# facebookresearch/vggsfm

Measured on NVIDIA H100. Metric: BA iterations/sec, higher is better.
Workload: dtype f64

## Files before the change

vggsfm_b200/csrc/ba_schur.cu:

```cuda
#include <stddef.h>
#include <algorithm>
#include <vector>
#include "ba_obs.h"
#include "common.cuh"
#include "dev_probes.h"
#include "syrk_work.h"

namespace vgg {

__device__ __forceinline__ void ar_add(double* local, double* mc, double v) {
  if (mc) asm volatile("multimem.red.relaxed.sys.global.add.f64 [%0], %1;" ::"l"(mc), "d"(v) : "memory");
  else atomicAdd(local, v);
}
__device__ __forceinline__ void ar_put(double* local, double* mc, double v) {
  if (mc) asm volatile("multimem.red.relaxed.sys.global.add.f64 [%0], %1;" ::"l"(mc), "d"(v) : "memory");
  else *local = v;
}

__global__ void jacobi_scale_points_kernel(int N, const double* __restrict__ H_pp, double* __restrict__ sc_p, int enable) {
  const int n = blockIdx.x * blockDim.x + threadIdx.x;
  if (n >= N) return;
  const double* h = H_pp + (size_t)n * 6;
  sc_p[n * 3 + 0] = enable ? 1.0 / (1.0 + sqrt(h[0])) : 1.0;
  sc_p[n * 3 + 1] = enable ? 1.0 / (1.0 + sqrt(h[3])) : 1.0;
// ... 29 lines not shown
  const double d2 = fmin(fmax(v22, min_diag), max_diag);
  dpp[n * 3] = d0; dpp[n * 3 + 1] = d1; dpp[n * 3 + 2] = d2;
  v00 += d0 / radius; v11 += d1 / radius; v22 += d2 / radius;
  bool bad = !(v00 > 0.0);
  const double l00 = sqrt(v00);
  const double l10 = v01 / l00, l20 = v02 / l00;
  const double t11 = v11 - l10 * l10;
  bad = bad || !(t11 > 0.0);
  const double l11 = sqrt(t11);
  const double l21 = (v12 - l20 * l10) / l11;
  const double t22 = v22 - l20 * l20 - l21 * l21;
  bad = bad || !(t22 > 0.0);
  const double l22 = sqrt(t22);
  if (bad) {
    atomicAdd(&scal[6], 1.0);
#pragma unroll
    for (int i = 0; i < 9; ++i) Mo[i] = 0.0;
    q[n * 3] = q[n * 3 + 1] = q[n * 3 + 2] = 0.0;
    return;
  }
  const double i00 = 1.0 / l00, i11 = 1.0 / l11, i22 = 1.0 / l22;
  const double i10 = -l10 * i00 * i11;
  const double i21 = -l21 * i11 * i22;
  const double i20 = -(l20 * i00 + l21 * i10) * i22;
  const double m00 = s0 * i00, m01 = s0 * i10, m02 = s0 * i20;
  const double m11 = s1 * i11, m12 = s1 * i21;
  const double m22 = s2 * i22;
  Mo[0] = m00; Mo[1] = m01; Mo[2] = m02;
  Mo[3] = 0.0; Mo[4] = m11; Mo[5] = m12;
  Mo[6] = 0.0; Mo[7] = 0.0; Mo[8] = m22;
  const double g0 = g_p[n * 3], g1 = g_p[n * 3 + 1], g2 = g_p[n * 3 + 2];
  q[n * 3 + 0] = m00 * g0;
  q[n * 3 + 1] = m01 * g0 + m11 * g1;
  q[n * 3 + 2] = m02 * g0 + m12 * g1 + m22 * g2;
}

__global__ void assemble_hc_kernel(int S, int dc, int ns, int KR, int Dpad, const double* __restrict__ camrec,
                                   const double* __restrict__ shared_in, double* __restrict__ Sraw,
                                   double* __restrict__ rhs, double* __restrict__ hdiag, double* __restrict__ gvec,
                                   ptrdiff_t mc_off) {
  const int s = blockIdx.x;
  const int tid = threadIdx.x;
#define VGG_PUT(ptr, val) ar_put((ptr), mc_off ? (ptr) + mc_off : nullptr, (val))
  if (s < S) {
    const double* rec = camrec + (size_t)s * KR;
    const int base = s * dc;
    if (tid < dc) {
      VGG_PUT(&gvec[base + tid], rec[tid]);
      VGG_PUT(&rhs[base + tid], -rec[tid]);
    }
    if (tid < dc * dc) {
      const int i = tid / dc, j = tid % dc;
      const int a = i < j ? i : j, b = i < j ? j : i;
      const int idx = dc + a * dc - a * (a - 1) / 2 + (b - a);
      const double val = rec[idx];
      VGG_PUT(&Sraw[(size_t)(base + i) * Dpad + base + j], val);
      if (i == j) VGG_PUT(&hdiag[base + i], val);
    }
    if (tid < 6 * ns) {
      const int i = tid / ns, j = tid % ns;
      const double val = rec[dc + dc * (dc + 1) / 2 + tid];
      VGG_PUT(&Sraw[(size_t)(S * dc + j) * Dpad + base + i], val);
      VGG_PUT(&Sraw[(size_t)(base + i) * Dpad + S * dc + j], val);
    }
  } else if (ns > 0) {
    const int base = S * dc;
    if (tid < ns) {
      VGG_PUT(&gvec[base + tid], shared_in[tid]);
      VGG_PUT(&rhs[base + tid], -shared_in[tid]);
    }
    if (tid < ns * ns) {
      const int i = tid / ns, j = tid % ns;
      const int a = i < j ? i : j, b = i < j ? j : i;
      const double val = shared_in[2 + (a == 0 ? b : 2)];
      VGG_PUT(&Sraw[(size_t)(base + i) * Dpad + base + j], val);
      if (i == j) VGG_PUT(&hdiag[base + i], val);
    }
  }
#undef VGG_PUT
}

constexpr int ZB_NT = 8;
constexpr int ZB_W = 4;
template <int MODEL, int MODE>
__global__ void __launch_bounds__(ZB_W * 32) z_build_kernel(
    int S, int N, int Dpad, const float* __restrict__ uv, const uint8_t* __restrict__ mask,
    const double* __restrict__ poses, const double* __restrict__ intr, const double* __restrict__ points,
    const uint8_t* __restrict__ point_const, const double* __restrict__ M, const double* __restrict__ q,
    double* __restrict__ Zt, double* __restrict__ rhs, ptrdiff_t mc_off, const int* __restrict__ fg_tracks) {
  using C = BlkCfg<MODEL, MODE>;
  constexpr int DC = C::DC, NS = C::NS;
  constexpr int ZR = 32 * DC;
  __shared__ __align__(16) double s_cam[ZB_W][16 * 32];
  __shared__ __align__(16) double s_z[ZB_W][3 * ZR];
  __shared__ double s_pt[ZB_NT][16];
  __shared__ double s_ws[ZB_W][ZB_NT][3 * (NS > 0 ? NS : 1)];
  const int lane = threadIdx.x & 31, warp = threadIdx.x >> 5;
  const int n0 = blockIdx.x * ZB_NT, nt = min(ZB_NT, N - n0);
  const int ngroups = (S + 31) / 32;
  for (int e = threadIdx.x; e < ZB_NT * 16; e += blockDim.x) {
    const int t = e >> 4, k = e & 15, n = n0 + t;
    double v = 0.0;
    if (t < nt) {
      if (k < 3) v = points[(size_t)n * 3 + k];
      else if (k == 3) v = (point_const && point_const[n]) ? 1.0 : 0.0;
      else if (k < 13) v = M[(size_t)n * 9 + (k - 4)];
      else v = q[(size_t)n * 3 + (k - 13)];
    }
    s_pt[t][k] = v;
  }
  if (NS > 0)
    for (int e = threadIdx.x; e < ZB_W * ZB_NT * 3 * NS; e += blockDim.x) (&s_ws[0][0][0])[e] = 0.0;
  __syncthreads();
  double* pw = s_cam[warp];
  double* zs = s_z[warp];
  const float2* uv2 = reinterpret_cast<const float2*>(uv);
  for (int g = warp; g < ngroups; g += ZB_W) {
    if (fg_tracks && (n0 + nt <= fg_tracks[2 * g] || n0 >= fg_tracks[2 * g + 1])) continue;
    const int s = g * 32 + lane;
    const bool frame_ok = s < S;
    const int cnt = min(32, S - g * 32) * DC;
    __syncwarp();
#pragma unroll
    for (int i = 0; i < 12; ++i) pw[i * 32 + lane] = frame_ok ? poses[(size_t)s * 12 + i] : 0.0;
#pragma unroll
    for (int i = 0; i < 4; ++i) pw[(12 + i) * 32 + lane] = frame_ok ? intr[(size_t)s * 4 + i] : 0.0;
    __syncwarp();
    double zq[DC];
#pragma unroll
    for (int i = 0; i < DC; ++i) zq[i] = 0.0;
    for (int t = 0; t < nt; ++t) {
      const size_t o = (size_t)s * N + n0 + t;
      const bool valid = frame_ok && mask[o] != 0;
      if (!__any_sync(0xffffffffu, valid)) continue;
      const float2 ob = frame_ok ? uv2[o] : make_float2(0.f, 0.f);
      const double* pt = s_pt[t];
      const double* m = pt + 4;
      double jc0[8], jc1[8], jx0[3], jx1[3], rx, ry;
      obs_math<MODEL>(pw + lane, 32, pt[0], pt[1], pt[2], pt[3] != 0.0, ob.x, ob.y, valid, jc0, jc1, jx0, jx1, rx, ry);
#pragma unroll
      for (int i = 0; i < DC; ++i) {
        const double w0 = w_entry(jc0, jc1, jx0, jx1, i, 0), w1 = w_entry(jc0, jc1, jx0, jx1, i, 1),
                     w2 = w_entry(jc0, jc1, jx0, jx1, i, 2);
        const double z0 = w0 * m[0];
        const double z1 = w0 * m[1] + w1 * m[4];
        const double z2 = w0 * m[2] + w1 * m[5] + w2 * m[8];
        zs[lane * DC + i] = z0;
        zs[ZR + lane * DC + i] = z1;
        zs[2 * ZR + lane * DC + i] = z2;
        zq[i] += z0 * m[9] + z1 * m[10] + z2 * m[11];
      }
      if (NS > 0) {
        double a[8];
#pragma unroll
        for (int k = 0; k < 8; ++k) a[k] = k < 3 * NS ? w_entry(jc0, jc1, jx0, jx1, 6 + k / 3, k % 3) : 0.0;
        const double r = warp_reduce_scatter<8>(a, lane);
        if (lane < 3 * NS) s_ws[warp][t][lane] += r;
      }
      __syncwarp();
      double* dst = Zt + (size_t)(3 * (n0 + t)) * Dpad + (size_t)g * ZR;
#pragma unroll
      for (int c = 0; c < 3; ++c, dst += Dpad) {
        const double* src = zs + c * ZR;
        for (int e = 2 * lane; e + 1 < cnt; e += 64)
          *reinterpret_cast<double2*>(dst + e) = *reinterpret_cast<const double2*>(src + e);
        if ((cnt & 1) && lane == 0) dst[cnt - 1] = src[cnt - 1];
      }
      __syncwarp();
    }
    if (frame_ok) {
#pragma unroll
      for (int i = 0; i < DC; ++i) {
        double* r = &rhs[(size_t)s * DC + i];
        if (zq[i] != 0.0) ar_add(r, mc_off ? r + mc_off : nullptr, zq[i]);
      }
    }
  }
  if (NS > 0) {
    __syncthreads();
    if ((int)threadIdx.x < nt * NS) {
      const int t = threadIdx.x / NS, j = threadIdx.x % NS;
      double w[3];
#pragma unroll
      for (int c = 0; c < 3; ++c) {
        w[c] = 0.0;
#pragma unroll
        for (int v = 0; v < ZB_W; ++v) w[c] += s_ws[v][t][j * 3 + c];
      }
      const double* m = s_pt[t] + 4;
      const double z0 = w[0] * m[0];
      const double z1 = w[0] * m[1] + w[1] * m[4];
      const double z2 = w[0] * m[2] + w[1] * m[5] + w[2] * m[8];
      double* zo = Zt + (size_t)(3 * (n0 + t)) * Dpad + (size_t)S * DC + j;
      zo[0] = z0;
      zo[Dpad] = z1;
      zo[2 * (size_t)Dpad] = z2;
      const double zq = z0 * m[9] + z1 * m[10] + z2 * m[11];
      double* r = &rhs[(size_t)S * DC + j];
      if (zq != 0.0) ar_add(r, mc_off ? r + mc_off : nullptr, zq);
    }
  }
}

constexpr int SF_BM = 128, SF_BK = 16, SF_LDS = 132, SF_STAGES = 4, SF_MMA_WARPS = 8;
constexpr int SF_THREADS = 128 + SF_MMA_WARPS * 32;
constexpr int SF_STAGE_DOUBLES = 2 * SF_BK * SF_LDS;
constexpr size_t SF_SMEM_BYTES = sizeof(double) * SF_STAGES * SF_STAGE_DOUBLES + sizeof(uint64_t) * 2 * SF_STAGES;

struct SyrkWork {
  int bi, bj, kb0, kb1;
};

__global__ void __launch_bounds__(SF_THREADS, 1)
    syrk_f64_kernel(const SyrkWork* __restrict__ work, int nwork, int Kpad, int Dpad, const double* __restrict__ Zt,
                    double* __restrict__ Cmat, ptrdiff_t mc_off, const __grid_constant__ FabricDev fd) {
  extern __shared__ __align__(16) double sf_smem[];
  uint64_t* full = reinterpret_cast<uint64_t*>(sf_smem + SF_STAGES * SF_STAGE_DOUBLES);
  uint64_t* empty = full + SF_STAGES;
  const int warp = threadIdx.x >> 5, lane = threadIdx.x & 31;
  if (threadIdx.x == 0) {
    for (int s = 0; s < SF_STAGES; ++s) {
      mbar_init(&full[s], 1);
      mbar_init(&empty[s], SF_MMA_WARPS);
    }
    mbar_fence_init();
  }
  __syncthreads();

  int stage = 0, phase = 0;
  if (warp < 4) {
    asm volatile("setmaxnreg.dec.sync.aligned.u32 40;");
    if (warp > 0) return;
    const int row = lane & (SF_BK - 1), opnd = lane / SF_BK;
    for (int w = blockIdx.x; w < nwork; w += gridDim.x) {
      const SyrkWork wk = work[w];
      const bool diag = wk.bi == wk.bj;
      const int k1 = min(Kpad, wk.kb1 * 64);
      for (int k = wk.kb0 * 64; k < k1; k += SF_BK) {
        mbar_wait(&empty[stage], phase ^ 1);
        if (lane == 0) mbar_expect_tx(&full[stage], (diag ? 1u : 2u) * SF_BK * SF_BM * (uint32_t)sizeof(double));
        __syncwarp();
        if (opnd == 0 || !diag)
          tma_load_1d(sf_smem + stage * SF_STAGE_DOUBLES + (opnd * SF_BK + row) * SF_LDS,
                      Zt + (size_t)(k + row) * Dpad + (opnd ? wk.bj : wk.bi) * SF_BM, SF_BM * sizeof(double), &full[stage]);
        if (++stage == SF_STAGES) {
          stage = 0;
          phase ^= 1;
        }
      }
    }
    return;
  }

  asm volatile("setmaxnreg.inc.sync.aligned.u32 232;");
  const int wm = (warp - 4) >> 2, wn = warp & 3;
  const int g = lane >> 2, t = lane & 3;
  for (int w = blockIdx.x; w < nwork; w += gridDim.x) {
// ... 220 lines not shown
      Q[i * 4 + j] = rot ? E[i * 3] * P[j] + E[i * 3 + 1] * P[4 + j] + E[i * 3 + 2] * P[8 + j] : P[i * 4 + j];
  Q[3] = d[3] != 0.0 ? P[3] + d[3] : P[3];
  Q[7] = d[4] != 0.0 ? P[7] + d[4] : P[7];
  Q[11] = d[5] != 0.0 ? P[11] + d[5] : P[11];
  const int ni = (model == VGG_SIMPLE_PINHOLE) ? 1 : 2;
  double f = intr[s * 4], k = intr[s * 4 + 3];
  const double* di = dc > 6 ? d + 6 : d_c + (size_t)S * dc;
  if (dc > 6 || ns > 0) {
    if (di[0] != 0.0) f += di[0];
    if (ni > 1 && di[1] != 0.0) k += di[1];
  }
  intr_c[s * 4] = f;
  intr_c[s * 4 + 1] = intr[s * 4 + 1];
  intr_c[s * 4 + 2] = intr[s * 4 + 2];
  intr_c[s * 4 + 3] = k;
}

__global__ void extract_gvec_kernel(int S, int dc, int ns, int KR, const double* __restrict__ camrec,
                                    const double* __restrict__ shared_in, double* __restrict__ gvec) {
  const int i = blockIdx.x * blockDim.x + threadIdx.x;
  const int D = S * dc + ns;
  if (i >= D) return;
  gvec[i] = (i < S * dc) ? camrec[(size_t)(i / dc) * KR + (i % dc)] : shared_in[i - S * dc];
}

__global__ void gradmax_kernel(int D, int N, const double* __restrict__ gvec, const uint8_t* __restrict__ pconst,
                               const double* __restrict__ g_p, const uint8_t* __restrict__ point_const,
                               double* __restrict__ scal) {
  const int i = blockIdx.x * blockDim.x + threadIdx.x;
  unsigned long long mc = 0, mp = 0;
  if (i < D && !pconst[i]) mc = (unsigned long long)__double_as_longlong(fabs(gvec[i]));
  if (i < N * 3 && !(point_const && point_const[i / 3])) mp = (unsigned long long)__double_as_longlong(fabs(g_p[i]));
#pragma unroll
  for (int off = 16; off >= 1; off >>= 1) {
    mc = max(mc, __shfl_xor_sync(0xffffffffu, mc, off));
    mp = max(mp, __shfl_xor_sync(0xffffffffu, mp, off));
  }
  if ((threadIdx.x & 31) == 0) {
    atomicMax(reinterpret_cast<unsigned long long*>(&scal[4]), mc);
    atomicMax(reinterpret_cast<unsigned long long*>(&scal[5]), mp);
  }
}

int launch_jacobi_scale_points(int N, const double* H_pp, double* sc_p, int enable, cudaStream_t st) {
  jacobi_scale_points_kernel<<<(N + 255) / 256, 256, 0, st>>>(N, H_pp, sc_p, enable);
  VGG_LAUNCH_CHECK();
  return VGG_OK;
}
int launch_jacobi_scale_cams(int D, const double* hdiag, double* sc_c, int enable, cudaStream_t st) {
  jacobi_scale_cams_kernel<<<(D + 255) / 256, 256, 0, st>>>(D, hdiag, sc_c, enable);
  VGG_LAUNCH_CHECK();
  return VGG_OK;
}
int launch_point_prep(int N, const double* H_pp, const double* g_p, const double* sc_p, const uint8_t* point_const,
                      double radius, double min_diag, double max_diag, double* M, double* q, double* dpp,
                      double* scal, cudaStream_t st) {
  point_prep_kernel<<<(N + 127) / 128, 128, 0, st>>>(N, H_pp, g_p, sc_p, point_const, radius, min_diag, max_diag, M, q,
                                                     dpp, scal);
  VGG_LAUNCH_CHECK();
  return VGG_OK;
}
int launch_assemble_hc(int S, int dc, int ns, int KR, int Dpad, const double* camrec, const double* shared_in,
                       double* Sraw, double* rhs, double* hdiag, double* gvec, ptrdiff_t mc_off, cudaStream_t st) {
  assemble_hc_kernel<<<S + (ns > 0 ? 1 : 0), 64, 0, st>>>(S, dc, ns, KR, Dpad, camrec, shared_in, Sraw, rhs, hdiag, gvec,
                                                          mc_off);
  VGG_LAUNCH_CHECK();
  return VGG_OK;
}
#define VGG_PICK_BA_KERNEL(kern, tmpl, p)                 \
  decltype(&tmpl<0, 0>) kern = nullptr;                   \
  switch ((p)->camera_model * 3 + (p)->intr_mode) {       \
    case 0: kern = tmpl<0, 0>; break;                     \
    case 1: kern = tmpl<0, 1>; break;                     \
    case 2: kern = tmpl<0, 2>; break;                     \
    case 3: kern = tmpl<1, 0>; break;                     \
    case 4: kern = tmpl<1, 1>; break;                     \
    case 5: kern = tmpl<1, 2>; break;                     \
  }                                                       \
  VGG_REQUIRE(kern, "bad camera_model/intr_mode")

int launch_z_build(const vgg_ba_problem* p, int Dpad, const double* M, const double* q, double* Zt, double* rhs,
                   ptrdiff_t mc_off, const int* fg_tracks, cudaStream_t st) {
  VGG_PICK_BA_KERNEL(kern, z_build_kernel, p);
  const int nw = std::min(ZB_W, (p->S + 31) / 32);
  kern<<<(p->N + ZB_NT - 1) / ZB_NT, nw * 32, 0, st>>>(p->S, p->N, Dpad, p->uv, p->mask, p->poses, p->intr, p->points,
                                                        p->point_const, M, q, Zt, rhs, mc_off, fg_tracks);
  VGG_LAUNCH_CHECK();
  return VGG_OK;
}

struct SyrkF64State {
  int dev = -1, Kpad = -1, Dpad = -1, sms = 0, nwork = 0;
  std::vector<int> ranges;
  SyrkWork* work_dev = nullptr;
  size_t work_cap = 0;
};
thread_local SyrkF64State g_sf;

static std::vector<SyrkWork> syrk_f64_work(int Kpad, int Dpad, const std::vector<int>& ranges, int nworkers) {
  const int nb = Dpad / SF_BM, KB = (Kpad + 63) / 64;
  std::vector<SyrkWork> work;
  build_work_list<SyrkWork>({1}, syrk_tile_jobs(nb, ranges), KB, nworkers, KB, 1,
                            [](const SyrkTileJob& j, int, int k0, int k1) { return SyrkWork{j.bi, j.bj, k0, k1}; }, &work);
  return work;
}

int launch_syrk(int Kpad, int Dpad, const double* Zt, double* Cmat, ptrdiff_t mc_off, const std::vector<int>& kb_ranges,
                const FabricDev& fd, cudaStream_t st) {
  VGG_REQUIRE(Dpad % SF_BM == 0 && Kpad % SF_BK == 0, "syrk: Dpad must be a multiple of 128 and Kpad of 16");
  const int nb = Dpad / SF_BM;
  SyrkF64State& hs = g_sf;
  const std::vector<int> ranges = (int)kb_ranges.size() == 2 * nb ? kb_ranges : std::vector<int>();
  int dev = 0;
  VGG_CUDA_CHECK(cudaGetDevice(&dev));
  if (hs.dev != dev || hs.Kpad != Kpad || hs.Dpad != Dpad || hs.ranges != ranges) {
    VGG_CUDA_CHECK(cudaDeviceGetAttribute(&hs.sms, cudaDevAttrMultiProcessorCount, dev));
    VGG_CUDA_CHECK(cudaFuncSetAttribute(syrk_f64_kernel, cudaFuncAttributeMaxDynamicSharedMemorySize, (int)SF_SMEM_BYTES));
    const std::vector<SyrkWork> work = syrk_f64_work(Kpad, Dpad, ranges, hs.sms);
    VGG_CUDA_CHECK(cudaDeviceSynchronize());
    if (hs.dev != dev || work.size() > hs.work_cap) {
      if (hs.work_dev) cudaFree(hs.work_dev);
      hs.work_dev = nullptr;
      hs.work_cap = std::max<size_t>(work.size(), 1);
      VGG_CUDA_CHECK(cudaMalloc(reinterpret_cast<void**>(&hs.work_dev), sizeof(SyrkWork) * hs.work_cap));
    }
    if (!work.empty())
      VGG_CUDA_CHECK(cudaMemcpy(hs.work_dev, work.data(), sizeof(SyrkWork) * work.size(), cudaMemcpyHostToDevice));
    hs.nwork = (int)work.size();
    hs.dev = dev;
    hs.Kpad = Kpad;
    hs.Dpad = Dpad;
    hs.ranges = ranges;
  }
  if (hs.nwork == 0) return VGG_OK;
  syrk_f64_kernel<<<std::min(hs.sms, hs.nwork), SF_THREADS, SF_SMEM_BYTES, st>>>(hs.work_dev, hs.nwork, Kpad, Dpad, Zt, Cmat,
                                                                               mc_off, fd);
  VGG_LAUNCH_CHECK();
  return VGG_OK;
}
int launch_scale_damp(int D, int Dpad, double* A, const double* rhs, const double* hdiag, const double* sc,
                      const uint8_t* pconst, double radius, double min_diag, double max_diag, double* bvec,
                      cudaStream_t st) {
  dim3 grid((D + 255) / 256, D);
  scale_damp_kernel<<<grid, 256, 0, st>>>(D, Dpad, A, rhs, hdiag, sc, pconst, radius, min_diag, max_diag, bvec);
  VGG_LAUNCH_CHECK();
  return VGG_OK;
}
int launch_cam_step(int D, const double* dcs, size_t dcs_stride, const double* sc, const double* hdiag, const double* gvec,
                    const uint8_t* pconst, double radius, double min_diag, double max_diag, double* d_c, double* scal,
                    cudaStream_t st) {
  cam_step_kernel<<<(D + 255) / 256, 256, 0, st>>>(D, dcs, dcs_stride, sc, hdiag, gvec, pconst, radius, min_diag, max_diag, d_c, scal);
  VGG_LAUNCH_CHECK();
  return VGG_OK;
}
int launch_backsub(const vgg_ba_problem* p, const double* d_c, double* wacc, const int* fg_tracks, cudaStream_t st) {
  VGG_PICK_BA_KERNEL(kern, backsub_kernel, p);
  const int nw = std::min(BS_W, p->S);
  kern<<<(p->N + 31) / 32, nw * 32, 0, st>>>(p->S, p->N, p->uv, p->mask, p->poses, p->intr, p->points, p->point_const,
                                             d_c, wacc, fg_tracks);
  VGG_LAUNCH_CHECK();
  return VGG_OK;
}
int launch_point_step(int N, const double* M, const double* g_p, const double* wacc, const double* sc_p,
                      const double* dpp, const uint8_t* point_const, const double* X, double radius, double* Xc,
                      double* scal, cudaStream_t st) {
  point_step_kernel<<<(N + 127) / 128, 128, 0, st>>>(N, M, g_p, wacc, sc_p, dpp, point_const, X, radius, Xc, scal);
  VGG_LAUNCH_CHECK();
  return VGG_OK;
// ... 61 lines not shown
```

vggsfm_b200/csrc/trsv.cu:

```cuda
#include "common.cuh"
#include "dev_probes.h"

namespace vgg {

namespace {

constexpr int TS_NB = 64;
constexpr int TS_THREADS = 256;
constexpr unsigned long long TS_SENTINEL = 0xffffffffffffffffull;

__global__ void __launch_bounds__(TS_THREADS, 1)
    trsv_upper_kernel(int n, int lda, const double* __restrict__ A, const double* __restrict__ y, size_t y_stride,
                      double* __restrict__ x, long long* __restrict__ stamps) {
  extern __shared__ __align__(16) double ts_smem[];
  double(*Ud)[TS_NB + 1] = reinterpret_cast<double(*)[TS_NB + 1]>(ts_smem);
  double(*Vi)[TS_NB + 1] = reinterpret_cast<double(*)[TS_NB + 1]>(ts_smem + TS_NB * (TS_NB + 1));
  double* xs = ts_smem + 2 * TS_NB * (TS_NB + 1);
  double* accs = xs + TS_NB;
  const int nb = gridDim.x;
  const int b = nb - 1 - (int)blockIdx.x;
  const int r0 = b * TS_NB;
  const int rows = min(TS_NB, n - r0);
  const int tid = threadIdx.x;
  const int r = tid >> 2, seg = tid & 3;
  auto stamp = [&](int k) {
    if (stamps && tid == 0) {
      long long t;
      asm volatile("mov.u64 %0, %%globaltimer;" : "=l"(t));
      stamps[6 * b + k] = t;
    }
  };
  stamp(0);
  double y_mine = 0.0;
  if (tid < TS_NB && tid < rows) y_mine = __ldcg(&y[(size_t)(r0 + tid) * y_stride]);

  for (int e = tid; e < TS_NB * TS_NB; e += TS_THREADS) {
    const int i = e / TS_NB, j = e % TS_NB;
    double v = (i == j) ? 1.0 : 0.0;
    if (i < rows && j < rows && j >= i) v = A[(size_t)(r0 + i) * lda + r0 + j];
    Ud[i][j] = v;
  }
  __syncthreads();
  stamp(1);
  if (tid < TS_NB) xs[tid] = 1.0 / Ud[tid][tid];
  __syncthreads();
  {
    const int c = tid >> 2, part = tid & 3;
    for (int i = TS_NB - 1; i >= 0; --i) {
      double s = 0.0;
      if (i < c) {
        for (int k = i + 1 + part; k <= c; k += 4) s = fma(-Ud[i][k], Vi[k][c], s);
      }
      s += __shfl_xor_sync(0xffffffffu, s, 1);
      s += __shfl_xor_sync(0xffffffffu, s, 2);
      if (part == 0) Vi[i][c] = i > c ? 0.0 : (i == c ? xs[i] : s * xs[i]);
      __syncwarp();
    }
  }
  __syncthreads();
  stamp(2);
  if (tid < TS_NB) accs[tid] = y_mine;
  __syncthreads();
  stamp(5);

  double t0[16], t1[16], t2[16];
  auto load_tile = [&](double (&tile)[16], int j) {
    const int c0 = j * TS_NB + seg * 16;
    const double* src = A + (size_t)(r0 + (r < rows ? r : 0)) * lda + c0;
#pragma unroll
    for (int k = 0; k < 16; ++k) tile[k] = (j > b && r < rows && c0 + k < n) ? src[k] : 0.0;
  };
  double acc = 0.0;
  auto hop = [&](const double (&tile)[16], int j) {
    if (tid < TS_NB) {
      double v = 0.0;
      if (j * TS_NB + tid < n) {
        const volatile unsigned long long* src = reinterpret_cast<const volatile unsigned long long*>(&x[j * TS_NB + tid]);
        unsigned long long bits;
        do {
          bits = *src;
        } while (bits == TS_SENTINEL);
        v = __longlong_as_double((long long)bits);
      }
      xs[tid] = v;
    }
    __syncthreads();
    double s0 = 0.0, s1 = 0.0, s2 = 0.0, s3 = 0.0;
#pragma unroll
    for (int k = 0; k < 16; k += 4) {
      s0 = fma(tile[k], xs[seg * 16 + k], s0);
      s1 = fma(tile[k + 1], xs[seg * 16 + k + 1], s1);
      s2 = fma(tile[k + 2], xs[seg * 16 + k + 2], s2);
      s3 = fma(tile[k + 3], xs[seg * 16 + k + 3], s3);
    }
    acc += (s0 + s1) + (s2 + s3);
    __syncthreads();
  };
  int j = nb - 1;
  if (b < nb - 1) {
  load_tile(t0, j);
  load_tile(t1, j - 1);
  load_tile(t2, j - 2);
  while (j > b) {
    hop(t0, j);
    load_tile(t0, j - 3);
    if (--j <= b) break;
    hop(t1, j);
    load_tile(t1, j - 3);
    if (--j <= b) break;
    hop(t2, j);
    load_tile(t2, j - 3);
    --j;
  }
  }
  stamp(3);
  acc += __shfl_xor_sync(0xffffffffu, acc, 1);
  acc += __shfl_xor_sync(0xffffffffu, acc, 2);
  if (seg == 0) accs[r] -= acc;
  __syncthreads();
  {
    double q0 = 0.0, q1 = 0.0, q2 = 0.0, q3 = 0.0;
#pragma unroll
    for (int k = 0; k < 16; k += 4) {
      const int c = seg * 16 + k;
      q0 = fma(c >= r ? Vi[r][c] : 0.0, accs[c], q0);
      q1 = fma(c + 1 >= r ? Vi[r][c + 1] : 0.0, accs[c + 1], q1);
      q2 = fma(c + 2 >= r ? Vi[r][c + 2] : 0.0, accs[c + 2], q2);
      q3 = fma(c + 3 >= r ? Vi[r][c + 3] : 0.0, accs[c + 3], q3);
    }
    double s = (q0 + q1) + (q2 + q3);
    s += __shfl_xor_sync(0xffffffffu, s, 1);
    s += __shfl_xor_sync(0xffffffffu, s, 2);
    if (seg == 0 && r < rows) {
      unsigned long long bits = (unsigned long long)__double_as_longlong(s);
      if (s != s) bits = 0x7ff8000000000000ull;
      *reinterpret_cast<volatile unsigned long long*>(&x[r0 + r]) = bits;
    }
  }
  if (stamps) {
    __syncthreads();
    stamp(4);
  }
}

}

int launch_trsv_upper(int n, int lda, const double* A, const double* y, size_t y_stride, double* x, long long* stamps,
                      cudaStream_t st) {
  const int nb = (n + TS_NB - 1) / TS_NB;
  VGG_REQUIRE(nb <= 120, "trsv_upper: n too large for one co-resident wave");
  const size_t smem = sizeof(double) * (2 * TS_NB * (TS_NB + 1) + 2 * TS_NB);
  static bool attr = false;
  if (!attr) {
    VGG_CUDA_CHECK(cudaFuncSetAttribute(trsv_upper_kernel, cudaFuncAttributeMaxDynamicSharedMemorySize, (int)smem));
    attr = true;
  }
  VGG_CUDA_CHECK(cudaMemsetAsync(x, 0xFF, sizeof(double) * (size_t)n, st));
  trsv_upper_kernel<<<nb, TS_THREADS, smem, st>>>(n, lda, A, y, y_stride, x, stamps);
  VGG_LAUNCH_CHECK();
  return VGG_OK;
}

}

extern "C" int vgg_dev_trsv_probe(int n, int lda, const double* A_dev, const double* y_dev, size_t y_stride, double* x_dev,
                                  long long* stamps_host) {
  using namespace vgg;
  VGG_REQUIRE(n > 0 && lda >= n && A_dev && y_dev && x_dev && y_stride > 0, "bad argument");
  const int nb = (n + TS_NB - 1) / TS_NB;
  static long long* d = nullptr;
  static int d_cap = 0;
  if (stamps_host && d_cap < 6 * nb) {
    if (d) cudaFree(d);
    VGG_CUDA_CHECK(cudaMalloc(&d, sizeof(long long) * 6 * nb));
    d_cap = 6 * nb;
  }
  if (stamps_host) VGG_CUDA_CHECK(cudaMemset(d, 0, sizeof(long long) * 6 * nb));
  const int rc = launch_trsv_upper(n, lda, A_dev, y_dev, y_stride, x_dev, stamps_host ? d : nullptr, 0);
  if (rc) return rc;
  VGG_CUDA_CHECK(cudaDeviceSynchronize());
  if (stamps_host) VGG_CUDA_CHECK(cudaMemcpy(stamps_host, d, sizeof(long long) * 6 * nb, cudaMemcpyDeviceToHost));
  return VGG_OK;
}
```

Before: 373.6.

## Rewrite TRSV as a 16-CTA cluster kernel with TMA ring and DSMEM broadcast

The blocked upper-triangular solve moves from one CTA per block row, which spin-polled global memory for sentinel values, to a single 16-CTA thread-block cluster. Each CTA owns strided block rows and streams off-diagonal tiles through a TMA-fed multi-stage shared-memory ring. Solved x segments are broadcast to every CTA with st.async into distributed shared memory, signalled by mbarriers, and diagonal blocks are inverted with a recursive doubling scheme. Separately, z_build now makes the four warps of a block share camera groups and split the tracks between them, staging observations in shared memory and reducing rhs contributions before the atomics. The cluster size of 16 needs the non-portable cluster attribute, and shared memory capacity limits n.

```diff
diff --git a/vggsfm_b200/csrc/ba_schur.cu b/vggsfm_b200/csrc/ba_schur.cu
--- a/vggsfm_b200/csrc/ba_schur.cu
+++ b/vggsfm_b200/csrc/ba_schur.cu
@@ -135,6 +135,7 @@
 
 constexpr int ZB_NT = 8;
 constexpr int ZB_W = 4;
+constexpr int ZB_TW = ZB_NT / ZB_W;
 template <int MODEL, int MODE>
 __global__ void __launch_bounds__(ZB_W * 32) z_build_kernel(
     int S, int N, int Dpad, const float* __restrict__ uv, const uint8_t* __restrict__ mask,
@@ -144,10 +145,13 @@
   using C = BlkCfg<MODEL, MODE>;
   constexpr int DC = C::DC, NS = C::NS;
   constexpr int ZR = 32 * DC;
-  __shared__ __align__(16) double s_cam[ZB_W][16 * 32];
+  __shared__ __align__(16) double s_cam[16 * 32];
   __shared__ __align__(16) double s_z[ZB_W][3 * ZR];
+  __shared__ double s_zq[ZB_W][32 * DC];
   __shared__ double s_pt[ZB_NT][16];
   __shared__ double s_ws[ZB_W][ZB_NT][3 * (NS > 0 ? NS : 1)];
+  __shared__ float2 s_ob[ZB_W][ZB_TW][32];
+  __shared__ uint8_t s_mk[ZB_W][ZB_TW][32];
   const int lane = threadIdx.x & 31, warp = threadIdx.x >> 5;
   const int n0 = blockIdx.x * ZB_NT, nt = min(ZB_NT, N - n0);
   const int ngroups = (S + 31) / 32;
@@ -165,28 +169,46 @@
   if (NS > 0)
     for (int e = threadIdx.x; e < ZB_W * ZB_NT * 3 * NS; e += blockDim.x) (&s_ws[0][0][0])[e] = 0.0;
   __syncthreads();
-  double* pw = s_cam[warp];
+  const double* pw = s_cam;
   double* zs = s_z[warp];
   const float2* uv2 = reinterpret_cast<const float2*>(uv);
-  for (int g = warp; g < ngroups; g += ZB_W) {
+  const int tw0 = warp * ZB_TW;
+  for (int g = 0; g < ngroups; ++g) {
     if (fg_tracks && (n0 + nt <= fg_tracks[2 * g] || n0 >= fg_tracks[2 * g + 1])) continue;
     const int s = g * 32 + lane;
     const bool frame_ok = s < S;
     const int cnt = min(32, S - g * 32) * DC;
-    __syncwarp();
-#pragma unroll
-    for (int i = 0; i < 12; ++i) pw[i * 32 + lane] = frame_ok ? poses[(size_t)s * 12 + i] : 0.0;
-#pragma unroll
-    for (int i = 0; i < 4; ++i) pw[(12 + i) * 32 + lane] = frame_ok ? intr[(size_t)s * 4 + i] : 0.0;
-    __syncwarp();
+    __syncthreads();
+    for (int e = threadIdx.x; e < 16 * 32; e += ZB_W * 32) {
+      const int i = e >> 5, fs = g * 32 + (e & 31);
+      s_cam[e] = fs < S ? (i < 12 ? poses[(size_t)fs * 12 + i] : intr[(size_t)fs * 4 + (i - 12)]) : 0.0;
+    }
+    {
+      uint8_t mk[ZB_TW];
+      float2 ob[ZB_TW];
+#pragma unroll
+      for (int k = 0; k < ZB_TW; ++k) {
+        const size_t o = (size_t)s * N + n0 + tw0 + k;
+        const bool in = frame_ok && tw0 + k < nt;
+        mk[k] = in ? mask[o] : (uint8_t)0;
+        ob[k] = in ? uv2[o] : make_float2(0.f, 0.f);
+      }
+#pragma unroll
+      for (int k = 0; k < ZB_TW; ++k) {
+        s_mk[warp][k][lane] = mk[k];
+        s_ob[warp][k][lane] = ob[k];
+      }
+    }
+    __syncthreads();
     double zq[DC];
 #pragma unroll
     for (int i = 0; i < DC; ++i) zq[i] = 0.0;
-    for (int t = 0; t < nt; ++t) {
-      const size_t o = (size_t)s * N + n0 + t;
-      const bool valid = frame_ok && mask[o] != 0;
+#pragma unroll 1
+    for (int k = 0; k < ZB_TW && tw0 + k < nt; ++k) {
+      const int t = tw0 + k;
+      const bool valid = s_mk[warp][k][lane] != 0;
       if (!__any_sync(0xffffffffu, valid)) continue;
-      const float2 ob = frame_ok ? uv2[o] : make_float2(0.f, 0.f);
+      const float2 ob = s_ob[warp][k][lane];
       const double* pt = s_pt[t];
       const double* m = pt + 4;
       double jc0[8], jc1[8], jx0[3], jx1[3], rx, ry;
@@ -206,7 +228,7 @@
       if (NS > 0) {
         double a[8];
 #pragma unroll
-        for (int k = 0; k < 8; ++k) a[k] = k < 3 * NS ? w_entry(jc0, jc1, jx0, jx1, 6 + k / 3, k % 3) : 0.0;
+        for (int kk = 0; kk < 8; ++kk) a[kk] = kk < 3 * NS ? w_entry(jc0, jc1, jx0, jx1, 6 + kk / 3, kk % 3) : 0.0;
         const double r = warp_reduce_scatter<8>(a, lane);
         if (lane < 3 * NS) s_ws[warp][t][lane] += r;
       }
@@ -221,11 +243,16 @@
       }
       __syncwarp();
     }
-    if (frame_ok) {
-#pragma unroll
-      for (int i = 0; i < DC; ++i) {
-        double* r = &rhs[(size_t)s * DC + i];
-        if (zq[i] != 0.0) ar_add(r, mc_off ? r + mc_off : nullptr, zq[i]);
+#pragma unroll
+    for (int i = 0; i < DC; ++i) s_zq[warp][lane * DC + i] = zq[i];
+    __syncthreads();
+    for (int e = threadIdx.x; e < 32 * DC; e += ZB_W * 32) {
+      double v = 0.0;
+#pragma unroll
+      for (int w = 0; w < ZB_W; ++w) v += s_zq[w][e];
+      if (g * 32 + e / DC < S && v != 0.0) {
+        double* r = &rhs[(size_t)g * 32 * DC + e];
+        ar_add(r, mc_off ? r + mc_off : nullptr, v);
       }
     }
   }
@@ -612,8 +639,7 @@
 int launch_z_build(const vgg_ba_problem* p, int Dpad, const double* M, const double* q, double* Zt, double* rhs,
                    ptrdiff_t mc_off, const int* fg_tracks, cudaStream_t st) {
   VGG_PICK_BA_KERNEL(kern, z_build_kernel, p);
-  const int nw = std::min(ZB_W, (p->S + 31) / 32);
-  kern<<<(p->N + ZB_NT - 1) / ZB_NT, nw * 32, 0, st>>>(p->S, p->N, Dpad, p->uv, p->mask, p->poses, p->intr, p->points,
+  kern<<<(p->N + ZB_NT - 1) / ZB_NT, ZB_W * 32, 0, st>>>(p->S, p->N, Dpad, p->uv, p->mask, p->poses, p->intr, p->points,
                                                         p->point_const, M, q, Zt, rhs, mc_off, fg_tracks);
   VGG_LAUNCH_CHECK();
   return VGG_OK;
diff --git a/vggsfm_b200/csrc/trsv.cu b/vggsfm_b200/csrc/trsv.cu
--- a/vggsfm_b200/csrc/trsv.cu
+++ b/vggsfm_b200/csrc/trsv.cu
@@ -1,3 +1,6 @@
+#include <cuda.h>
+#include <cudaTypedefs.h>
+#include <algorithm>
 #include "common.cuh"
 #include "dev_probes.h"
 
@@ -7,140 +10,256 @@
 
 constexpr int TS_NB = 64;
 constexpr int TS_THREADS = 256;
-constexpr unsigned long long TS_SENTINEL = 0xffffffffffffffffull;
+constexpr int TC_CS = 16;
+constexpr int TC_TILE = TS_NB * TS_NB;
+constexpr int TC_MAX_STAGES = 8;
+constexpr size_t TC_SMEM_MAX = 227 * 1024;
+
+__host__ __device__ constexpr size_t tc_fixed_bytes(int nb) {
+  return sizeof(double) * (2 * TS_NB * (TS_NB + 1) + (size_t)nb * TS_NB + (size_t)((nb + TC_CS - 1) / TC_CS) * TS_NB) +
+         8 * ((size_t)nb + TC_MAX_STAGES) + 128;
+}
+
+__device__ __forceinline__ uint32_t cluster_rank() {
+  uint32_t r;
+  asm volatile("mov.u32 %0, %%cluster_ctarank;" : "=r"(r));
+  return r;
+}
+__device__ __forceinline__ void cluster_sync() {
+  asm volatile("barrier.cluster.arrive.release.aligned;\n\tbarrier.cluster.wait.acquire.aligned;" ::: "memory");
+}
+__device__ __forceinline__ uint32_t mapa(uint32_t saddr, uint32_t rank) {
+  uint32_t r;
+  asm volatile("mapa.shared::cluster.u32 %0, %1, %2;" : "=r"(r) : "r"(saddr), "r"(rank));
+  return r;
+}
+__device__ __forceinline__ void st_async_f64(uint32_t addr, double v, uint32_t bar) {
+  asm volatile("st.async.shared::cluster.mbarrier::complete_tx::bytes.b64 [%0], %1, [%2];" ::"r"(addr),
+               "l"((unsigned long long)__double_as_longlong(v)), "r"(bar)
+               : "memory");
+}
+__device__ __forceinline__ void mbar_wait_cluster(uint64_t* bar, uint32_t parity) {
+  uint32_t done = 0;
+  for (long spins = 0; !done && spins < (1L << 22); ++spins) {
+    asm volatile(
+        "{\n"
+        ".reg .pred p;\n"
+        "mbarrier.try_wait.parity.acquire.cluster.shared::cta.b64 p, [%1], %2;\n"
+        "selp.u32 %0, 1, 0, p;\n"
+        "}\n"
+        : "=r"(done)
+        : "r"(smem_u32(bar)), "r"(parity)
+        : "memory");
+  }
+}
+
+__device__ __forceinline__ void tc_stamp(long long* stamps, int b, int k) {
+  if (stamps && threadIdx.x == 0) {
+    long long t;
+    asm volatile("mov.u64 %0, %%globaltimer;" : "=l"(t));
+    stamps[6 * b + k] = t;
+  }
+}
+
+__device__ __noinline__ void tc_invert(int n, int lda, const double* __restrict__ A, int b, double (*Ud)[TS_NB + 1],
+                                       double (*Vi)[TS_NB + 1], long long* stamps) {
+  const int tid = threadIdx.x;
+  const int r0 = b * TS_NB, rows = min(TS_NB, n - r0);
+  for (int e = tid; e < TS_NB * TS_NB; e += TS_THREADS) {
+    const int i = e / TS_NB, jj = e % TS_NB;
+    double v = (i == jj) ? 1.0 : 0.0;
+    if (i < rows && jj < rows && jj >= i) v = A[(size_t)(r0 + i) * lda + r0 + jj];
+    Ud[i][jj] = v;
+    Vi[i][jj] = 0.0;
+  }
+  __syncthreads();
+  tc_stamp(stamps, b, 1);
+  if (tid < TS_NB) {
+    const int o = tid & ~7, cc = tid & 7;
+    double v[8];
+#pragma unroll
+    for (int i = 7; i >= 0; --i) {
+      double s = 0.0;
+#pragma unroll
+      for (int k = i + 1; k < 8; ++k) s = k <= cc ? fma(Ud[o + i][o + k], v[k], s) : s;
+      const double d = 1.0 / Ud[o + i][o + i];
+      v[i] = i > cc ? 0.0 : (i == cc ? d : -s * d);
+    }
+#pragma unroll
+    for (int i = 0; i < 8; ++i)
+      if (i <= cc) Vi[o + i][o + cc] = v[i];
+  }
+  __syncthreads();
+#pragma unroll 1
+  for (int h = 8; h < TS_NB; h *= 2) {
+    const int nout = (TS_NB / (2 * h)) * h * h;
+    double t[4];
+#pragma unroll
+    for (int u = 0; u < 4; ++u) {
+      const int o = tid + u * TS_THREADS;
+      t[u] = 0.0;
+      if (o < nout) {
+        const int p = o / (h * h), i = (o / h) % h, j = o % h, base = p * 2 * h;
+        double s = 0.0;
+        for (int k = 0; k <= j; ++k) s = fma(Ud[base + i][base + h + k], Vi[base + h + k][base + h + j], s);
+        t[u] = s;
+      }
+    }
+    __syncthreads();
+#pragma unroll
+    for (int u = 0; u < 4; ++u) {
+      const int o = tid + u * TS_THREADS;
+      if (o < nout) {
+        const int p = o / (h * h), i = (o / h) % h, j = o % h, base = p * 2 * h;
+        Ud[base + i][base + h + j] = t[u];
+      }
+    }
+    __syncthreads();
+#pragma unroll
+    for (int u = 0; u < 4; ++u) {
+      const int o = tid + u * TS_THREADS;
+      if (o < nout) {
+        const int p = o / (h * h), i = (o / h) % h, j = o % h, base = p * 2 * h;
+        double s = 0.0;
+        for (int k = i; k < h; ++k) s = fma(Vi[base + i][base + k], Ud[base + k][base + h + j], s);
+        Vi[base + i][base + h + j] = -s;
+      }
+    }
+    __syncthreads();
+  }
+  tc_stamp(stamps, b, 2);
+}
 
 __global__ void __launch_bounds__(TS_THREADS, 1)
-    trsv_upper_kernel(int n, int lda, const double* __restrict__ A, const double* __restrict__ y, size_t y_stride,
-                      double* __restrict__ x, long long* __restrict__ stamps) {
-  extern __shared__ __align__(16) double ts_smem[];
-  double(*Ud)[TS_NB + 1] = reinterpret_cast<double(*)[TS_NB + 1]>(ts_smem);
-  double(*Vi)[TS_NB + 1] = reinterpret_cast<double(*)[TS_NB + 1]>(ts_smem + TS_NB * (TS_NB + 1));
-  double* xs = ts_smem + 2 * TS_NB * (TS_NB + 1);
-  double* accs = xs + TS_NB;
-  const int nb = gridDim.x;
-  const int b = nb - 1 - (int)blockIdx.x;
-  const int r0 = b * TS_NB;
-  const int rows = min(TS_NB, n - r0);
+    trsv_cluster_kernel(int n, int lda, const double* __restrict__ A, const double* __restrict__ y, size_t y_stride,
+                        double* __restrict__ x, int nst, const __grid_constant__ CUtensorMap tmap,
+                        long long* __restrict__ stamps) {
+  extern __shared__ __align__(16) double ts_raw[];
+  double* ts_smem = ts_raw + ((128 - (smem_u32(ts_raw) & 127)) & 127) / sizeof(double);
+  const int nb = (n + TS_NB - 1) / TS_NB;
+  const int q = (int)cluster_rank();
+  double* ring = ts_smem;
+  double(*Ud)[TS_NB + 1] = reinterpret_cast<double(*)[TS_NB + 1]>(ring + (size_t)nst * TC_TILE);
+  double(*Vi)[TS_NB + 1] = Ud + TS_NB;
+  double* xs = &Vi[0][0] + TS_NB * (TS_NB + 1);
+  double* accs = xs + (size_t)nb * TS_NB;
+  uint64_t* bars = reinterpret_cast<uint64_t*>(accs + (size_t)((nb + TC_CS - 1) / TC_CS) * TS_NB);
+  uint64_t* full = bars + nb;
   const int tid = threadIdx.x;
   const int r = tid >> 2, seg = tid & 3;
-  auto stamp = [&](int k) {
-    if (stamps && tid == 0) {
-      long long t;
-      asm volatile("mov.u64 %0, %%globaltimer;" : "=l"(t));
-      stamps[6 * b + k] = t;
-    }
-  };
-  stamp(0);
-  double y_mine = 0.0;
-  if (tid < TS_NB && tid < rows) y_mine = __ldcg(&y[(size_t)(r0 + tid) * y_stride]);
-
-  for (int e = tid; e < TS_NB * TS_NB; e += TS_THREADS) {
-    const int i = e / TS_NB, j = e % TS_NB;
-    double v = (i == j) ? 1.0 : 0.0;
-    if (i < rows && j < rows && j >= i) v = A[(size_t)(r0 + i) * lda + r0 + j];
-    Ud[i][j] = v;
-  }
-  __syncthreads();
-  stamp(1);
-  if (tid < TS_NB) xs[tid] = 1.0 / Ud[tid][tid];
-  __syncthreads();
-  {
-    const int c = tid >> 2, part = tid & 3;
-    for (int i = TS_NB - 1; i >= 0; --i) {
-      double s = 0.0;
-      if (i < c) {
-        for (int k = i + 1 + part; k <= c; k += 4) s = fma(-Ud[i][k], Vi[k][c], s);
-      }
-      s += __shfl_xor_sync(0xffffffffu, s, 1);
-      s += __shfl_xor_sync(0xffffffffu, s, 2);
-      if (part == 0) Vi[i][c] = i > c ? 0.0 : (i == c ? xs[i] : s * xs[i]);
-      __syncwarp();
-    }
-  }
-  __syncthreads();
-  stamp(2);
-  if (tid < TS_NB) accs[tid] = y_mine;
-  __syncthreads();
-  stamp(5);
-
-  double t0[16], t1[16], t2[16];
-  auto load_tile = [&](double (&tile)[16], int j) {
-    const int c0 = j * TS_NB + seg * 16;
-    const double* src = A + (size_t)(r0 + (r < rows ? r : 0)) * lda + c0;
-#pragma unroll
-    for (int k = 0; k < 16; ++k) tile[k] = (j > b && r < rows && c0 + k < n) ? src[k] : 0.0;
-  };
-  double acc = 0.0;
-  auto hop = [&](const double (&tile)[16], int j) {
-    if (tid < TS_NB) {
-      double v = 0.0;
-      if (j * TS_NB + tid < n) {
-        const volatile unsigned long long* src = reinterpret_cast<const volatile unsigned long long*>(&x[j * TS_NB + tid]);
-        unsigned long long bits;
-        do {
-          bits = *src;
-        } while (bits == TS_SENTINEL);
-        v = __longlong_as_double((long long)bits);
-      }
-      xs[tid] = v;
-    }
+  const int rg = tid >> 4, cl = tid & 15;
+  const int top = nb - 1 - q;
+  const int nown = top >= 0 ? top / TC_CS + 1 : 0;
+  auto owned = [&](int m) { return top - m * TC_CS; };
+  auto stamp = [&](int b, int k) { tc_stamp(stamps, b, k); };
+#pragma unroll 1
+  for (int m = 0; m < nown; ++m) stamp(owned(m), 0);
+
+  for (int j = tid; j < nb; j += TS_THREADS) {
+    mbar_init(&bars[j], 1);
+    mbar_expect_tx(&bars[j], TS_NB * sizeof(double));
+  }
+  if (tid < nst) mbar_init(&full[tid], 1);
+  mbar_fence_init();
+  if (tid < TS_NB) {
+    for (int m = 0; m < nown; ++m) {
+      const int row = owned(m) * TS_NB + tid;
+      accs[m * TS_NB + tid] = row < n ? __ldcg(&y[(size_t)row * y_stride]) : 0.0;
+    }
+  }
+
+  auto finalize = [&](int m) {
+    const int b = owned(m), r0 = b * TS_NB;
     __syncthreads();
-    double s0 = 0.0, s1 = 0.0, s2 = 0.0, s3 = 0.0;
-#pragma unroll
-    for (int k = 0; k < 16; k += 4) {
-      s0 = fma(tile[k], xs[seg * 16 + k], s0);
-      s1 = fma(tile[k + 1], xs[seg * 16 + k + 1], s1);
-      s2 = fma(tile[k + 2], xs[seg * 16 + k + 2], s2);
-      s3 = fma(tile[k + 3], xs[seg * 16 + k + 3], s3);
-    }
-    acc += (s0 + s1) + (s2 + s3);
-    __syncthreads();
-  };
-  int j = nb - 1;
-  if (b < nb - 1) {
-  load_tile(t0, j);
-  load_tile(t1, j - 1);
-  load_tile(t2, j - 2);
-  while (j > b) {
-    hop(t0, j);
-    load_tile(t0, j - 3);
-    if (--j <= b) break;
-    hop(t1, j);
-    load_tile(t1, j - 3);
-    if (--j <= b) break;
-    hop(t2, j);
-    load_tile(t2, j - 3);
-    --j;
-  }
-  }
-  stamp(3);
-  acc += __shfl_xor_sync(0xffffffffu, acc, 1);
-  acc += __shfl_xor_sync(0xffffffffu, acc, 2);
-  if (seg == 0) accs[r] -= acc;
-  __syncthreads();
-  {
+    stamp(b, 3);
+    const double* ac = accs + m * TS_NB;
     double q0 = 0.0, q1 = 0.0, q2 = 0.0, q3 = 0.0;
 #pragma unroll
     for (int k = 0; k < 16; k += 4) {
       const int c = seg * 16 + k;
-      q0 = fma(c >= r ? Vi[r][c] : 0.0, accs[c], q0);
-      q1 = fma(c + 1 >= r ? Vi[r][c + 1] : 0.0, accs[c + 1], q1);
-      q2 = fma(c + 2 >= r ? Vi[r][c + 2] : 0.0, accs[c + 2], q2);
-      q3 = fma(c + 3 >= r ? Vi[r][c + 3] : 0.0, accs[c + 3], q3);
+      q0 = fma(Vi[r][c], ac[c], q0);
+      q1 = fma(Vi[r][c + 1], ac[c + 1], q1);
+      q2 = fma(Vi[r][c + 2], ac[c + 2], q2);
+      q3 = fma(Vi[r][c + 3], ac[c + 3], q3);
     }
     double s = (q0 + q1) + (q2 + q3);
     s += __shfl_xor_sync(0xffffffffu, s, 1);
     s += __shfl_xor_sync(0xffffffffu, s, 2);
-    if (seg == 0 && r < rows) {
-      unsigned long long bits = (unsigned long long)__double_as_longlong(s);
-      if (s != s) bits = 0x7ff8000000000000ull;
-      *reinterpret_cast<volatile unsigned long long*>(&x[r0 + r]) = bits;
-    }
-  }
-  if (stamps) {
-    __syncthreads();
-    stamp(4);
-  }
+    if (seg == 0 && r0 + r < n) x[r0 + r] = s;
+    const uint32_t xa = smem_u32(&xs[r0 + r]), ba = smem_u32(&bars[b]);
+#pragma unroll
+    for (int d = seg; d < TC_CS; d += 4) st_async_f64(mapa(xa, d), s, mapa(ba, d));
+    if (stamps) {
+      __syncthreads();
+      stamp(b, 4);
+    }
+  };
+
+  auto m_lo = [&](int j) { return top - j < 0 ? 0 : (top - j) / TC_CS + 1; };
+  int pj = nb - 1, pm = m_lo(nb - 1);
+  if (pj < 1 || pm >= nown) pj = 0;
+  auto load_next = [&](int stage) {
+    if (pj >= 1 && tid == 0) {
+      mbar_expect_tx(&full[stage], TC_TILE * sizeof(double));
+      asm volatile(
+          "cp.async.bulk.tensor.2d.shared::cluster.global.mbarrier::complete_tx::bytes [%0], [%1, {%2, %3}], [%4];" ::"r"(
+              smem_u32(ring + (size_t)stage * TC_TILE)),
+          "l"(reinterpret_cast<uint64_t>(&tmap)), "r"(pj * TS_NB), "r"(owned(pm) * TS_NB), "r"(smem_u32(&full[stage]))
+          : "memory");
+    }
+    if (pj >= 1 && ++pm >= nown) {
+      --pj;
+      pm = pj >= 1 ? m_lo(pj) : nown;
+      if (pm >= nown) pj = 0;
+    }
+  };
+
+  if (nown > 0) tc_invert(n, lda, A, owned(0), Ud, Vi, stamps);
+#pragma unroll 1
+  for (int m = 0; m < nown; ++m) stamp(owned(m), 5);
+  cluster_sync();
+#pragma unroll 1
+  for (int st = 0; st < nst; ++st) load_next(st);
+
+  int it = 0;
+  for (int j = nb; j >= 1; --j) {
+    const bool col = j < nb;
+    double x0 = 0.0, x1 = 0.0, x2 = 0.0, x3 = 0.0;
+    if (col) {
+      mbar_wait_cluster(&bars[j], 0);
+      x0 = xs[j * TS_NB + cl], x1 = xs[j * TS_NB + cl + 16], x2 = xs[j * TS_NB + cl + 32], x3 = xs[j * TS_NB + cl + 48];
+    }
+    for (int m = m_lo(j); m < nown; ++m) {
+      if (col) {
+        const int stage = it % nst;
+        mbar_wait(&full[stage], (uint32_t)(it / nst) & 1u);
+        const double* t = ring + (size_t)stage * TC_TILE + rg * TS_NB + cl;
+        double p[4];
+#pragma unroll
+        for (int i = 0; i < 4; ++i) {
+          const double* ti = t + i * 16 * TS_NB;
+          p[i] = fma(ti[0], x0, ti[16] * x1) + fma(ti[32], x2, ti[48] * x3);
+        }
+#pragma unroll
+        for (int off = 8; off >= 1; off >>= 1) {
+#pragma unroll
+          for (int i = 0; i < 4; ++i) p[i] += __shfl_xor_sync(0xffffffffu, p[i], off);
+        }
+        if (cl == 0) {
+#pragma unroll
+          for (int i = 0; i < 4; ++i) accs[m * TS_NB + rg + 16 * i] -= p[i];
+        }
+        ++it;
+        __syncthreads();
+        load_next(stage);
+      }
+      if (owned(m) == j - 1) {
+        finalize(m);
+        if (m + 1 < nown) tc_invert(n, lda, A, owned(m + 1), Ud, Vi, stamps);
+      }
+    }
+  }
+  mbar_wait_cluster(&bars[0], 0);
 }
 
 }
@@ -148,15 +267,44 @@
 int launch_trsv_upper(int n, int lda, const double* A, const double* y, size_t y_stride, double* x, long long* stamps,
                       cudaStream_t st) {
   const int nb = (n + TS_NB - 1) / TS_NB;
-  VGG_REQUIRE(nb <= 120, "trsv_upper: n too large for one co-resident wave");
-  const size_t smem = sizeof(double) * (2 * TS_NB * (TS_NB + 1) + 2 * TS_NB);
+  VGG_REQUIRE(lda % 2 == 0 && ((uintptr_t)A & 15) == 0, "trsv_upper: A must be 16-byte aligned with an even lda");
+  static PFN_cuTensorMapEncodeTiled_v12000 encode = nullptr;
+  if (!encode) {
+    cudaDriverEntryPointQueryResult qr;
+    VGG_CUDA_CHECK(cudaGetDriverEntryPoint("cuTensorMapEncodeTiled", (void**)&encode, cudaEnableDefault, &qr));
+    VGG_REQUIRE(qr == cudaDriverEntryPointSuccess && encode, "trsv_upper: cuTensorMapEncodeTiled unavailable");
+  }
+  CUtensorMap tmap;
+  const cuuint64_t dims[2] = {(cuuint64_t)n, (cuuint64_t)n};
+  const cuuint64_t strides[1] = {(cuuint64_t)lda * sizeof(double)};
+  const cuuint32_t box[2] = {TS_NB, TS_NB}, estr[2] = {1, 1};
+  VGG_REQUIRE(encode(&tmap, CU_TENSOR_MAP_DATA_TYPE_FLOAT64, 2, const_cast<double*>(A), dims, strides, box, estr,
+                     CU_TENSOR_MAP_INTERLEAVE_NONE, CU_TENSOR_MAP_SWIZZLE_NONE, CU_TENSOR_MAP_L2_PROMOTION_L2_256B,
+                     CU_TENSOR_MAP_FLOAT_OOB_FILL_NONE) == CUDA_SUCCESS,
+              "trsv_upper: tensor map encoding failed");
+  const size_t fixed = tc_fixed_bytes(nb);
+  const int nst = fixed < TC_SMEM_MAX ? (int)std::min<size_t>(TC_MAX_STAGES, (TC_SMEM_MAX - fixed) / (sizeof(double) * TC_TILE)) : 0;
+  VGG_REQUIRE(nst >= 2, "trsv_upper: n too large for the cluster's shared memory");
+  const size_t smem = fixed + sizeof(double) * TC_TILE * (size_t)nst;
   static bool attr = false;
   if (!attr) {
-    VGG_CUDA_CHECK(cudaFuncSetAttribute(trsv_upper_kernel, cudaFuncAttributeMaxDynamicSharedMemorySize, (int)smem));
+    VGG_CUDA_CHECK(cudaFuncSetAttribute(trsv_cluster_kernel, cudaFuncAttributeMaxDynamicSharedMemorySize, (int)TC_SMEM_MAX));
+    VGG_CUDA_CHECK(cudaFuncSetAttribute(trsv_cluster_kernel, cudaFuncAttributeNonPortableClusterSizeAllowed, 1));
     attr = true;
   }
-  VGG_CUDA_CHECK(cudaMemsetAsync(x, 0xFF, sizeof(double) * (size_t)n, st));
-  trsv_upper_kernel<<<nb, TS_THREADS, smem, st>>>(n, lda, A, y, y_stride, x, stamps);
+  cudaLaunchConfig_t cfg = {};
+  cfg.gridDim = dim3(TC_CS);
+  cfg.blockDim = dim3(TS_THREADS);
+  cfg.dynamicSmemBytes = smem;
+  cfg.stream = st;
+  cudaLaunchAttribute at[1];
+  at[0].id = cudaLaunchAttributeClusterDimension;
+  at[0].val.clusterDim.x = TC_CS;
+  at[0].val.clusterDim.y = 1;
+  at[0].val.clusterDim.z = 1;
+  cfg.attrs = at;
+  cfg.numAttrs = 1;
+  VGG_CUDA_CHECK(cudaLaunchKernelEx(&cfg, trsv_cluster_kernel, n, lda, A, y, y_stride, x, nst, tmap, stamps));
   VGG_LAUNCH_CHECK();
   return VGG_OK;
 }
```

Result: faster. 382.4 (median of 6 runs) (+2.4%).
